# hccho2/Tacotron-Wavenet-Vocoder-Korean

Measured on AMD Instinct MI355X. Metric: WaveNet autoregressive audio samples/sec at 24 kHz, batch=8, higher is better.
Workload: dtype f32

## Files before the change

### tacotron-wavenet-vocoder-korean_amd/csrc/twv_wavenet_xcd.hip

```cpp
#include <hip/hip_runtime.h>
#include <stdint.h>
#include <string>
#include <type_traits>
#include "../../include/twv_amd.h"
#include "twv_layout.hpp"
#include "twv_math.hpp"
#include "twv_dev.hpp"
#include "twv_dpp.hpp"
#include "twv_categorical.hpp"
#include "twv_xcd.hpp"

using namespace twv;

#ifndef TWV_CHAIN_PAD
#define TWV_CHAIN_PAD 0
#endif
#ifndef TWV_WATCHDOG_LOG2
#define TWV_WATCHDOG_LOG2 21
#endif
#define TWV_STR2(x) #x
#define TWV_STR(x) TWV_STR2(x)
namespace {

typedef __attribute__((address_space(1))) unsigned long long gu64;
#define LDSU64(i) (((__attribute__((address_space(3))) volatile unsigned long long*)lds)[(i)])

typedef unsigned u32x2v __attribute__((ext_vector_type(2)));
typedef unsigned u32x4s __attribute__((ext_vector_type(4)));
constexpr int kAuxLoad = (int)(16u | 0x80000000u), kAuxStore = 0;
#ifndef TWV_XCD_KF
#define TWV_XCD_KF 1
#endif

__device__ __forceinline__ unsigned long long xb_load(rsrc_t rs, int uword, int lword)
{
    asm volatile("" ::: "memory");
    const u32x2v v = __builtin_amdgcn_raw_buffer_load_b64(rs, lword * 8, uword * 8, kAuxLoad);
    return ((unsigned long long)v.y << 32) | (unsigned long long)v.x;
}
__device__ __forceinline__ u32x4s xb_load2(rsrc_t rs, int uword, int lpair)
{
    asm volatile("" ::: "memory");
    return __builtin_amdgcn_raw_buffer_load_b128(rs, lpair * 16, uword * 8, kAuxLoad);
}
template <bool BAR> __device__ __forceinline__ unsigned long long xb_load_t(rsrc_t rs, int uword, int lword)
{
    if (BAR) asm volatile("" ::: "memory");
    return xb_load(rs, uword, lword);
}
__device__ __forceinline__ unsigned long long xbm_load(rsrc_t rs, int uword, int lword) { return xb_load_t<true>(rs, uword, lword); }
__device__ __forceinline__ u32x4s xbm_load2(rsrc_t rs, int uword, int lpair)
{
    asm volatile("" ::: "memory");
    return xb_load2(rs, uword, lpair);
}
__device__ __forceinline__ void xb_store(rsrc_t rs, int uword, int lword, unsigned tag, float v)
{
    __builtin_amdgcn_raw_buffer_store_b64(u32x2v{__float_as_uint(v), tag}, rs, lword * 8, uword * 8, kAuxStore);
    asm volatile("" ::: "memory");
}
__device__ __forceinline__ void xb_store2(rsrc_t rs, int uword, int lane, unsigned tag, float va, float vb)
{
    const u32x4s d = {__float_as_uint(va), tag, __float_as_uint(vb), tag};
    __builtin_amdgcn_raw_buffer_store_b128(d, rs, lane * 16, uword * 8, kAuxStore);
    asm volatile("s_nop 1" ::"v"(d) : "memory");
}
__device__ __forceinline__ unsigned g_tag(unsigned long long q) { return (unsigned)(q >> 32); }
__device__ __forceinline__ float g_val(unsigned long long q) { return __uint_as_float((unsigned)q); }

struct Poll {
    rsrc_t rs;
    int* status;
    int it;
    bool dead;
};
template <bool BAR = false>
__device__ __forceinline__ bool poll_tick(Poll& p, int code)
{
    if (p.dead) return false;
    if (((++p.it) & 63) == 0) {
        if (xb_load_t<BAR>(p.rs, (int)XcdExch::CTRL + 1, 0) != 0ull) { p.dead = true; return false; }
        if (p.it > (1 << TWV_WATCHDOG_LOG2)) {
            atomicMax(p.status, code);
            xb_store(p.rs, (int)XcdExch::CTRL + 1, 0, 1u, 0.0f);
            p.dead = true;
            return false;
        }
    }
    return true;
}
__device__ __forceinline__ void nap_until(unsigned long long target)
{
#pragma nounroll
    for (int i = 0; i < 4096 && __builtin_amdgcn_s_memtime() < target; ++i) __builtin_amdgcn_s_sleep(8);
}

__device__ __forceinline__ int lane_of_z(int k) { return ((k & 2) ? 16 : 0) + 2 * (k >> 2) + (k & 1); }
__device__ __forceinline__ int lane_of_x(int j) { return j < 16 ? j : 16 + j; }

struct ChainRegs { float wc[32]; float bd; };

#define XSTAMP(cond_, slot_) do { if ((INSTR & 1) && a.prof != nullptr && b == a.prof_stream && t < a.prof_steps && lane == 0 && (cond_)) a.prof[(long long)t * 64 + (slot_)] = wall_clock64(); } while (0)

#define WACC_DECL() unsigned long long wacc_[6] = {0, 0, 0, 0, 0, 0}, w0_ = 0, wt0_ = 0; if (INSTR & 4) wt0_ = __builtin_amdgcn_s_memtime()
#define WACC_T0() do { if (INSTR & 4) w0_ = __builtin_amdgcn_s_memtime(); } while (0)
#define WACC_T1(i_) do { if (INSTR & 4) wacc_[i_] += __builtin_amdgcn_s_memtime() - w0_; } while (0)
constexpr int kTraceStep = 2000;
#define WTRACE(cond_, slot_) do { if ((INSTR & 4) && a.prof != nullptr && t == kTraceStep && (cond_) && lane == 0) a.prof[2048 + (slot_)] = wall_clock64(); } while (0)
#define WACC_OUT(prof_, slot_, wave_) do { if ((INSTR & 4) && (prof_) != nullptr && (slot_) >= 0 && lane == 0) {                 \
        unsigned long long* o_ = (prof_) + (((slot_) * 8 + (wave_)) * 8);                                                        \
        o_[0] = __builtin_amdgcn_s_memtime() - wt0_;                                                                             \
        o_[1] = wacc_[0]; o_[2] = wacc_[1]; o_[3] = wacc_[2]; o_[4] = wacc_[3]; o_[5] = wacc_[4]; o_[6] = wacc_[5]; } } while (0)
#define XMARK(role_, stage_) do { if ((INSTR & 1) && lane == 0) xb_store(rs, (int)XcdExch::MARK + (role_) * 8 + (int)(threadIdx.x >> 6), 0, (unsigned)t + 1u, (float)(stage_)); } while (0)

enum { ROLE_CHAIN = 0, ROLE_SERVICE = 1, ROLE_SKIP0 = 2, ROLE_CONV0 = 10, ROLE_LC0 = 18 };
constexpr int kXcdStreamsPerXcd = kXcdStreams / 8;

struct XArgs {
    XcdLaunch p;
    int n_lc_wg, lc_lpw;
    int total_roles;
};

template <int NS> struct XStreams { rsrc_t rs[NS]; int b[NS]; };
__device__ __forceinline__ rsrc_t exch_rsrc(const XcdLaunch& a, int b)
{
    return __builtin_amdgcn_make_buffer_rsrc(a.exch + (long long)b * XcdExch::WORDS, 0, (int)(XcdExch::WORDS * 8), 0x00020000);
}
struct XLazyRs { const XcdLaunch* a; int xcc, ns; __device__ __forceinline__ rsrc_t operator[](int k) const { return exch_rsrc(*a, xcc + 8 * (k < ns ? k : 0)); } };
struct XLazyB { int xcc, ns; __device__ __forceinline__ int operator[](int k) const { return xcc + 8 * (k < ns ? k : 0); } };
template <int NS> struct XStreamsLazy { XLazyRs rs; XLazyB b; };
constexpr int kSkipLdsWords = 32 * 64;
constexpr int kConvLdsFloats = 16 * 64 + 64;

template <int INSTR, bool ALL, bool FORCED, bool SEG1, bool TWOSEG, int NC, bool ONEHOT = false, int HW = -1>
__device__ __forceinline__ void chain_role(const XArgs& xa, int b, rsrc_t rs)
{
    const XcdLaunch& a = xa.p;
    const Layout& L = a.lay;
    const int w = __builtin_amdgcn_readfirstlane(threadIdx.x >> 6), lane = threadIdx.x & 63;
    const int NL = L.NL, T = a.T;
    const bool use_bias = L.use_bias != 0, has_gc = L.G > 0, has_lc = L.L > 0;
    constexpr bool forced = FORCED;
    const int l0 = SEG1 ? kXcdSeg0Layers + 4 * w : (w < 6 ? 4 * w : 24 + 3 * (w - 6));
    const int lw0 = SEG1 ? 4 * w : l0;
    const int cap = SEG1 ? 4 : (w < 6 ? 4 : 3);
    int nl = NL - l0;
    nl = nl < 0 ? 0 : (nl > cap ? cap : nl);
    const int nlc = NC >= 0 ? NC : nl;
    const bool next_has = (l0 + nl < NL);
    const bool head = HW >= 0 ? (HW == 1) : (!SEG1 && (w == 7));
    const bool to_seg1 = TWOSEG && !SEG1 && w == 7 && next_has;
    constexpr bool two_seg = TWOSEG;
    if (nl == 0 && !head) return;
    const int oc = dpp_conv_out(lane), od = dpp_dense_out(lane);
    const ActCoef coef = act_coef(lane >= 32);
    float* stb = a.state + (long long)b * L.state_stride;
    Poll pl{rs, a.status, 0, false};
    constexpr int O_WD = 2048;

    ChainRegs W[4];
#pragma unroll
    for (int i = 0; i < 4; ++i) {
        if (i < nl) {
            const f32x4* src = reinterpret_cast<const f32x4*>(a.P + L.off_xl + (long long)(l0 + i) * kXcdXlFloats) + lane;
#pragma unroll
            for (int q = 0; q < 8; ++q) { const f32x4 v = src[q * 64]; W[i].wc[4 * q] = v.x; W[i].wc[4 * q + 1] = v.y; W[i].wc[4 * q + 2] = v.z; W[i].wc[4 * q + 3] = v.w; }
#pragma unroll
            for (int q = 0; q < 4; ++q) LDS4((O_WD >> 2) + ((lw0 + i) * 4 + q) * 64 + lane) = src[(8 + q) * 64];
            const f32x4 v = src[12 * 64];
            W[i].bd = dense_bias_init(lane, use_bias ? v.y : 0.0f);
        }
    }
    float ha = 0.0f, hb = 0.0f, first_in = 0.0f, b2v = 0.0f, s_lnl = 0.0f, s_tq = 0.0f, samp = 0.0f;
    float cp[4] = {0.0f, 0.0f, 0.0f, 0.0f};
    int q_prev = 0, q_valid = 0, samp_q = 0, first_q = 0;
    float w0row = 0.0f;
    double u_next = 0.0;
    const int chx = dpp_dense_out(lane);
    const bool sampler = head && !forced;
    const bool is15 = (lane & 15) == 15;
    auto causal_prepare = [&]() {
        const float t1 = __int_as_float(__builtin_amdgcn_update_dpp(0, __float_as_int(ha), 0x101, 0xf, 0xf, true));
        const float b0 = __int_as_float(__builtin_amdgcn_update_dpp(0, __float_as_int(hb), 0x150, 0xf, 0xf, true));
        ha = is15 ? b0 : t1;
        hb = __int_as_float(__builtin_amdgcn_update_dpp(0, __float_as_int(hb), 0x101, 0xf, 0xf, true));
        causal_partial_dpp(W[3].wc, ha, hb, cp);
    };
    auto noise = [&](int t) {
        const float* up = a.uniforms + ((long long)b * T + t) * (L.nr_mix + 1);
        const float u = lane <= L.nr_mix ? up[lane] : 0.5f;
        s_lnl = log_e(-log_e(u));
        const float uu = __shfl(u, L.nr_mix);
        s_tq = log_e(uu) - log_e(1.0f - uu);
    };
    if (head) {
        if constexpr (ONEHOT) {
            const int* meta = reinterpret_cast<const int*>(stb + L.st_meta);
            q_valid = __builtin_amdgcn_readfirstlane(meta[M_PREV_VALID]);
            q_prev = __builtin_amdgcn_readfirstlane(meta[M_QPREV]) & (L.Q - 1);
            w0row = a.P[L.off_causal + (long long)q_prev * 32 + chx];
            if (!forced) first_q = reinterpret_cast<const int*>(a.first_input)[b];
        } else {
            const f32x4* src = reinterpret_cast<const f32x4*>(a.P + L.off_xc) + lane;
#pragma unroll
            for (int q = 0; q < 8; ++q) { const f32x4 v = src[q * 64]; W[3].wc[4 * q] = v.x; W[3].wc[4 * q + 1] = v.y; W[3].wc[4 * q + 2] = v.z; W[3].wc[4 * q + 3] = v.w; }
            ha = stb[L.st_hist + (lane & 15)];
            hb = stb[L.st_hist + 16 + (lane & 15)];
            if (!forced) first_in = reinterpret_cast<const float*>(a.first_input)[b];
            if (sampler && use_bias && lane < L.O) b2v = a.P[L.off_b2 + lane];
            causal_prepare();
        }
// ... 41 lines not shown
            if (lane == 0) {
                if (sampler && t > 0) a.out[(long long)b * T + t - 1] = samp;
                xb_store(rs, (int)XcdExch::CTRL, 0, tag, 0.0f);
            }
            hb = is15 ? s_in : hb;
            if (t + 1 < T) causal_prepare();
            if (sampler) noise(t);
            }
            __builtin_amdgcn_s_setprio(0);
        }
        XMARK(SEG1 ? 30 : ROLE_CHAIN, 1);
        float pre[4] = {0.0f, 0.0f, 0.0f, 0.0f};
        if (nlc > 0) {
            pl.it = 0;
            for (;;) {
                bool ok = true;
#pragma unroll
                for (int i = 0; i < 4; ++i) {
                    if (i < nlc) {
                        const unsigned long long qp = xb_load(rs, (int)XcdExch::PG + (l0 + i) * 64, oc);
                        ok = ok && g_tag(qp) == tag;
                        pre[i] = g_val(qp);
                    }
                }
                if (__all(ok)) break;
                if (!poll_tick(pl, 31)) break;
                __builtin_amdgcn_s_sleep(4);
            }
            XSTAMP(!SEG1, 26 + w);
            XMARK(SEG1 ? 30 : ROLE_CHAIN, 2);
            if (in_period) nap_until(t_in + in_period - (in_period >> 4));
            unsigned long long q;
            pl.it = 0;
            if (SEG1 && w == 0) {
                for (;;) {
                    q = xb_load(rs, (int)XcdExch::SEG, lane);
                    if (__all(g_tag(q) == tag)) break;
                    if (!poll_tick(pl, 36)) break;
                }
            } else {
                for (;;) {
                    q = LDSU64(w * 64 + lane);
                    if (__all(g_tag(q) == tag)) break;
                    if (!poll_tick(pl, 33)) break;
                }
            }
            __builtin_amdgcn_s_setprio(3);
            X = g_val(q);
            now_in = __builtin_amdgcn_s_memtime();
            XSTAMP(true, (SEG1 ? 40 : 2) + w);
            XMARK(SEG1 ? 30 : ROLE_CHAIN, 3);
        }
        constexpr bool DEFER = ALL && !FORCED && !SEG1 && NC > 0 && HW == 0;
        float zs[4] = {0.0f, 0.0f, 0.0f, 0.0f}, xs[4] = {0.0f, 0.0f, 0.0f, 0.0f};
        auto run_layers = [&](auto nc) {
            constexpr int N = decltype(nc)::value;
#pragma unroll
            for (int i = 0; i < N; ++i) {
                float wd[16];
#pragma unroll
                for (int q = 0; q < 4; ++q) {
                    const f32x4 v = LDS4((O_WD >> 2) + ((lw0 + i) * 4 + q) * 64 + lane);
                    wd[4 * q] = v.x; wd[4 * q + 1] = v.y; wd[4 * q + 2] = v.z; wd[4 * q + 3] = v.w;
                }
                const float z = layer_front_dpp(W[i].wc, coef, X, pre[i]);
                if (DEFER) { zs[i] = z; xs[i] = X; }
                else xb_store2(rs, (int)XcdExch::ZX + (l0 + i) * 128, lane, tag, z, X);
                layer_back_dpp(wd, W[i].bd, z, X);
                if ((INSTR & 2) && a.dbg != nullptr && t < a.dbg_steps) {
                    float* dp = a.dbg + ((long long)b * a.dbg_steps + t) * ((long long)NL * 64 + L.Opad) + (long long)(l0 + i) * 64;
                    if (lane < 32) dp[dpp_z_index(lane)] = z;
                    if ((lane & 16) == 0) dp[32 + od] = X;
                }
            }
        };
        if constexpr (NC > 0) run_layers(std::integral_constant<int, NC>{});
        else {
            if (nl == 4) run_layers(std::integral_constant<int, 4>{});
            else if (nl == 3) run_layers(std::integral_constant<int, 3>{});
            else if (nl == 2) run_layers(std::integral_constant<int, 2>{});
            else if (nl == 1) run_layers(std::integral_constant<int, 1>{});
        }
        if (to_seg1) xb_store(rs, (int)XcdExch::SEG, lane, tag, X);
        else if (nlc > 0) LDSU64((next_has ? w + 1 : 9) * 64 + lane) = ((unsigned long long)tag << 32) | (unsigned long long)__float_as_uint(X);
        XSTAMP(DEFER && nl > 0, (SEG1 ? 48 : 10) + w);
        if (DEFER) {
#pragma unroll
            for (int i = 0; i < (NC > 0 ? NC : 0); ++i) xb_store2(rs, (int)XcdExch::ZX + (l0 + i) * 128, lane, tag, zs[i], xs[i]);
        }
        if (forced && nl > 0 && !next_has) {
            if (SEG1) xb_store(rs, (int)XcdExch::DONE, lane, tag, 0.0f);
            else LDSU64(8 * 64 + lane) = (unsigned long long)tag << 32;
        }
        if (nlc > 0) {
            const unsigned long long d = now_in - t_in;
            in_period = (t_in != 0 && d < (1ull << 18)) ? d : 0;
            t_in = now_in;
        }
        if (!sampler) __builtin_amdgcn_s_setprio(0);
        XSTAMP(!DEFER && nl > 0, (SEG1 ? 48 : 10) + w);
        XMARK(SEG1 ? 30 : ROLE_CHAIN, 4);
        if constexpr (ONEHOT) {
          if (sampler) {
            __builtin_amdgcn_s_setprio(3);
            u32x4s d0, d1;
            pl.it = 0;
            for (;;) {
                d0 = xb_load2(rs, (int)XcdExch::QL, lane * 2);
                d1 = xb_load2(rs, (int)XcdExch::QL, lane * 2 + 1);
                if (__all(d0.y == tag && d0.w == tag && d1.y == tag && d1.w == tag)) break;
                if (!poll_tick(pl, 34)) break;
            }
            XSTAMP(true, 18);
            XMARK(SEG1 ? 30 : ROLE_CHAIN, 5);
            const float y[4] = {__uint_as_float(d0.x), __uint_as_float(d0.z), __uint_as_float(d1.x), __uint_as_float(d1.z)};
            if ((INSTR & 2) && a.dbg != nullptr && t < a.dbg_steps) {
#pragma unroll
                for (int k = 0; k < 4; ++k)
                    a.dbg[((long long)b * a.dbg_steps + t) * ((long long)NL * 64 + L.Opad) + (long long)NL * 64 + lane + 64 * k] = y[k];
            }
            bool bad_p = false;
            samp_q = categorical_sample<4>(y, L.Q, lane, a.temperature, u_next, nullptr,
                                           ((INSTR & 1) && a.prof != nullptr && b == a.prof_stream && t < a.prof_steps) ? a.prof + (long long)t * 64 + 38 : nullptr, &bad_p);
            if (bad_p && lane == 0) atomicMax(a.status, 31);
            XSTAMP(true, 19);
          }
        } else
        if (sampler) {
            __builtin_amdgcn_s_setprio(3);
            const int half = lane >> 5;
            unsigned long long q[8];
            pl.it = 0;
            for (;;) {
                bool good = true;
#pragma unroll
                for (int k = 0; k < 4; ++k) {
                    const u32x4s d = xb_load2(rs, (int)XcdExch::PT, (half * 4 + k) * 32 + (lane & 31));
                    q[2 * k] = ((unsigned long long)d.y << 32) | d.x;
                    q[2 * k + 1] = ((unsigned long long)d.w << 32) | d.z;
                    good = good && d.y == tag && d.w == tag;
                }
                if (__all(good)) break;
                if (!poll_tick(pl, 34)) break;
            }
            XSTAMP(true, 18);
            XMARK(SEG1 ? 30 : ROLE_CHAIN, 5);
            float y = g_val(q[0]);
#pragma unroll
            for (int k = 1; k < 8; ++k) y = y + g_val(q[k]);
#pragma unroll
            for (int k = 0; k < 8; ++k) {
                const auto sw = __builtin_amdgcn_permlane32_swap((unsigned)q[k], (unsigned)q[k], false, false);
                y = y + __uint_as_float(sw[1]);
// ... 327 lines not shown
                        if (!summer) __builtin_amdgcn_s_sleep(1);
                    }
                    if ((INSTR & 1) && pl.dead && g == 0 && lane == 0) {
                        xb_store(rs, (int)XcdExch::MARK + 176 + v * 4, 0, g_tag(qz), __uint_as_float(g_tag(qz)));
                        xb_store(rs, (int)XcdExch::MARK + 177 + v * 4, 0, (unsigned)l, __uint_as_float((unsigned)pl.it));
                        xb_store(rs, (int)XcdExch::MARK + 178 + v * 4, 0, tag, __uint_as_float((unsigned)si));
                    }
                    if (!anysum && k == 0) {
                        const unsigned long long now = __builtin_amdgcn_s_memtime();
                        if (si == 0) { const unsigned long long d = now - seen[0]; period = (seen[0] != 0 && d < (1ull << 18)) ? d : 0; }
                        seen[si] = now;
                    }
                    XSTAMP(g == 0 && summer && l == NL - 1, 20);
                    const auto sw = __builtin_amdgcn_permlane32_swap((unsigned)qz, (unsigned)qz, false, false);
                    float val = dot(__uint_as_float(sw[0]), __uint_as_float(sw[1]));
                    if (use_bias) val = val + bias;
                    if (!summer) {
                        LDSU64(k * SW + l * 64 + lane) = ((unsigned long long)tag << 32) | (unsigned long long)__float_as_uint(val);
                    } else {
                        drain(true);
                        tot[k] = (l == 0) ? val : tot[k] + val;
                        nextl[k] = l + 1;
                        if (l == NL - 1 && !pl.dead) {
                            const float h = (KF > 0 || tot[k] > 0.0f) ? tot[k] : 0.0f;
                            xb_store(rs, (int)XcdExch::H1 + g * 64, lane, tag, h);
                            XSTAMP(g == 0, 21);
                        }
                    }
                }
            }
        };
#pragma unroll
        for (int j = 0; j < kLds; ++j) {
            if (j < nlds && !pl.dead)
                own_layer([&](float xa_, float xb_) __attribute__((always_inline)) { return dot32_dpp_lds(o_tile4 + (v + 8 * j) * (kTile / 4), lane, xa_, xb_); }, bs[j], v + 8 * j, j, 0, NS);
        }
#pragma unroll
        for (int i = 0; i < kReg; ++i) {
            if (i < nown && !pl.dead) {
                const int l = NLDS + v + 8 * i;
                own_layer([&](float xa_, float xb_) __attribute__((always_inline)) { return dot32_dpp(ws[i].w, xa_, xb_); }, bs[kLds + i], l, kLds + i, 0,
                          (SPLIT && vB >= 0 && l == NL - 1) ? 2 : NS);
            }
        }
        if (SPLIT && sumB && !pl.dead)
            own_layer([&](float xa_, float xb_) __attribute__((always_inline)) { return dot32_dpp(wx.w, xa_, xb_); }, bx, NL - 1, kSlots, 2, NS);
    }
    if (pl.dead && lane == 0) {
#pragma unroll
        for (int k = 0; k < NS; ++k) xb_store(sx.rs[k], (int)XcdExch::CTRL + 1, 0, 1u, 0.0f);
    }
}

template <int KF, bool BAR>
__device__ __forceinline__ unsigned long long conv1_fetch_h1(Poll& pl, const rsrc_t rs, const int v, const int lane, const unsigned tag, const int last_layer,
                                                             const int zc_lane, const float (&wl)[32], const float bl, const bool use_bias, bool& saw_z)
{
    unsigned long long q;
    pl.it = 0;
    if (KF > 0) {
        unsigned long long qz;
        float val = 0.0f;
        bool havez = false;
        for (;;) {
            if (!havez) qz = xb_load_t<BAR>(rs, (int)XcdExch::ZX + last_layer * 128, zc_lane * 2);
            q = xb_load_t<BAR>(rs, (int)XcdExch::H1 + v * 64, lane);
            if (!havez && __all(g_tag(qz) == tag)) {
                const auto sw = __builtin_amdgcn_permlane32_swap((unsigned)qz, (unsigned)qz, false, false);
                val = dot32_dpp(wl, __uint_as_float(sw[0]), __uint_as_float(sw[1]));
                if (use_bias) val = val + bl;
                havez = true;
                saw_z = true;
            }
            if (havez && __all(g_tag(q) == tag)) break;
            if (!poll_tick<BAR>(pl, 61)) break;
            if (!havez) __builtin_amdgcn_s_sleep(1);
        }
        const float tot = g_val(q) + val;
        const float h = tot > 0.0f ? tot : 0.0f;
        q = (unsigned long long)__float_as_uint(h);
    } else {
        for (;;) {
            q = xb_load_t<BAR>(rs, (int)XcdExch::H1 + v * 64, lane);
            if (__all(g_tag(q) == tag)) break;
            if (!poll_tick<BAR>(pl, 61)) break;
            __builtin_amdgcn_s_sleep(1);
        }
    }
    return q;
}
__device__ __forceinline__ void conv1_load_last_skip(const XcdLaunch& a, const int v, const int lane, Tile& wl, float& bl)
{
    const Layout& L = a.lay;
    const long long lb = L.off_layer0 + (long long)(L.NL - 1) * L.layer_stride;
    load_tile(wl, a.P + lb + LayerOff::SK + (long long)v * kTile, lane);
    if (L.use_bias != 0) bl = a.P[lb + LayerOff::SK + (long long)L.NSJ * kTile + v * 64 + lane];
}

template <int INSTR, int NS, bool BAR = false, class SX = XStreams<NS>, int KF = 0>
__device__ __forceinline__ void conv1_role(const XArgs& xa, const SX& sx, int g, const int ns_rt = NS, const int prof_slot = -1)
{
    const XcdLaunch& a = xa.p;
    const Layout& L = a.lay;
    const int v = __builtin_amdgcn_readfirstlane(threadIdx.x >> 6), lane = threadIdx.x & 63;
    const int T = a.T, NCH = L.NCH;
    const bool use_bias = L.use_bias != 0;
    Poll pl{sx.rs[0], a.status, 0, false};
    constexpr int O_PART = 0, O_CNT = 16 * 64;
    if (threadIdx.x < NS) LDSI(threadIdx.x * kConvLdsFloats + O_CNT) = 0;
    __syncthreads();
    const int c0 = 2 * v, c1 = 2 * v + 1;
    Tile ta, tb;
    load_tile(ta, a.P + L.off_w1 + ((long long)g * NCH + c0) * kTile, lane);
    load_tile(tb, a.P + L.off_w1 + ((long long)g * NCH + c1) * kTile, lane);
    const bool summer = v < 2;
    float b1v = 0.0f;
    Tile t2;
    if (summer) {
        if (use_bias) b1v = a.P[L.off_b1 + g * 64 + lane];
        load_tile(t2, a.P + L.off_w2 + (long long)(2 * g + v) * kTile, lane);
    }
    Tile wl;
    float bl = 0.0f;
    if (KF > 0) conv1_load_last_skip(a, v, lane, wl, bl);
    const int zc_lane = lane_of_z((lane < 32 ? 0 : 16) + (lane & 15));
    unsigned long long t_arr = 0, period = 0;
    WACC_DECL();
    for (int t = 0; t < T && !pl.dead; ++t) {
        asm volatile(".p2align 6");
        const unsigned tag = (unsigned)t + 1u;
        WACC_T0();
        if (period) nap_until(t_arr + period - (period >> 3));
        WACC_T1(0);
#pragma unroll
        for (int k = 0; k < NS; ++k) {
            if (pl.dead) break;
            if (k >= ns_rt) break;
            const rsrc_t rs = sx.rs[k];
            const int b = sx.b[k];
            const int ob = k * kConvLdsFloats;
            pl.rs = rs;
            XMARK(ROLE_CONV0 + g, 1);
            WACC_T0();
            bool saw_z = false;
            const unsigned long long q = conv1_fetch_h1<KF, BAR>(pl, rs, v, lane, tag, L.NL - 1, zc_lane, wl.w, bl, use_bias, saw_z);
            (void)saw_z;
            WACC_T1(1);
            WTRACE(prof_slot >= 0 && k == 0, 400 + g * 8 + v);
            unsigned long long now_arr = 0;
            if (k == 0) now_arr = __builtin_amdgcn_s_memtime();
            XSTAMP(g == 0 && v == 0, 22);
            const unsigned hq = (unsigned)q;
            const auto p16 = __builtin_amdgcn_permlane16_swap(hq, hq, false, false);
            const auto pa = __builtin_amdgcn_permlane32_swap(p16[0], p16[0], false, false);
            const auto pb = __builtin_amdgcn_permlane32_swap(p16[1], p16[1], false, false);
            float r0, r1;
            dot32_dpp_x2(ta.w, __uint_as_float(pa[0]), __uint_as_float(pb[0]), tb.w, __uint_as_float(pa[1]), __uint_as_float(pb[1]), r0, r1);
            lds[ob + O_PART + c0 * 64 + lane] = r0;
            lds[ob + O_PART + c1 * 64 + lane] = r1;
            asm volatile("" ::: "memory");
            if (lane == 0) __hip_atomic_fetch_add(&LDSI(ob + O_CNT), 1, __ATOMIC_RELAXED, __HIP_MEMORY_SCOPE_WORKGROUP);
            if (k == 0) {
                const unsigned long long d = now_arr - t_arr;
                period = (t_arr != 0 && d < (1ull << 18)) ? d : 0;
                t_arr = now_arr;
            }
            XSTAMP(g == 0 && v == 0, 23);
            XMARK(ROLE_CONV0 + g, 2);
            if (summer) {
                WACC_T0();
                pl.it = 0;
                while (LDSVI(ob + O_CNT) < 8 * (t + 1)) { if (!poll_tick<BAR>(pl, 62)) break; }
                WACC_T1(2);
                asm volatile("" ::: "memory");
                XSTAMP(g == 0 && v == 0, 24);
                float cp[16];
#pragma unroll
                for (int ch = 0; ch < 16; ++ch) cp[ch] = lds[ob + O_PART + ch * 64 + lane];
                __builtin_amdgcn_sched_barrier(0);
                float r = cp[0];
#pragma unroll
                for (int ch = 1; ch < 16; ++ch) r = r + cp[ch];
                if (use_bias) r = r + b1v;
                const float h = r > 0.0f ? r : 0.0f;
                const float p = (v == 0) ? dot_readlane_pipe(t2, h) : dot_readlane_pipe32(t2, h);
                if (lane < 32) xb_store(rs, (int)XcdExch::PT, (g * 32 + lane) * 2 + v, tag, p);
                WTRACE(prof_slot >= 0 && k == 0, 480 + g * 2 + v);
                XSTAMP(g == 0 && v == 0, 25);
            }
        }
    }
    if (pl.dead && lane == 0) {
#pragma unroll
        for (int k = 0; k < NS; ++k) xb_store(sx.rs[k], (int)XcdExch::CTRL + 1, 0, 1u, 0.0f);
    }
    WACC_OUT(a.prof, prof_slot, v);
}

constexpr int kConvQLdsFloats = 16 * 64 + 64 + 8 * 64;
template <int INSTR, int NS, int KF = 0>
__device__ __forceinline__ void conv1_onehot_role(const XArgs& xa, const XStreams<NS>& sx, int g)
{
    const XcdLaunch& a = xa.p;
    const Layout& L = a.lay;
    const int v = __builtin_amdgcn_readfirstlane(threadIdx.x >> 6), lane = threadIdx.x & 63;
    const int T = a.T, NCH = L.NCH;
    const bool use_bias = L.use_bias != 0;
    Poll pl{sx.rs[0], a.status, 0, false};
    constexpr int O_PART = 0, O_CNT = 16 * 64, O_P2 = 16 * 64 + 64;
    if (threadIdx.x < NS) { LDSI(threadIdx.x * kConvQLdsFloats + O_CNT) = 0; LDSI(threadIdx.x * kConvQLdsFloats + O_CNT + 1) = 0; }
    __syncthreads();
    const int c0 = 2 * v, c1 = 2 * v + 1;
    Tile ta, tb;
    load_tile(ta, a.P + L.off_w1 + ((long long)g * NCH + c0) * kTile, lane);
    load_tile(tb, a.P + L.off_w1 + ((long long)g * NCH + c1) * kTile, lane);
    float w2[32];
    {
        const int ch2 = lane < 32 ? c0 : c1;
        const f32x4* src = reinterpret_cast<const f32x4*>(a.P + L.off_w2 + ((long long)(g >> 1) * NCH + ch2) * kTile) + ((g & 1) * 32 + (lane & 31));
#pragma unroll
        for (int q = 0; q < 8; ++q) { const f32x4 w = src[q * 64]; w2[4 * q] = w.x; w2[4 * q + 1] = w.y; w2[4 * q + 2] = w.z; w2[4 * q + 3] = w.w; }
    }
    float b1v = 0.0f, b2v = 0.0f;
    if (use_bias && v == 0) b1v = a.P[L.off_b1 + g * 64 + lane];
    if (use_bias && v == 1 && lane < 32) b2v = a.P[L.off_b2 + g * 32 + lane];
    Tile wl;
    float bl = 0.0f;
    if (KF > 0) conv1_load_last_skip(a, v, lane, wl, bl);
    const int zc_lane = lane_of_z((lane < 32 ? 0 : 16) + (lane & 15));
    const int cls = g * 32 + (lane & 31);
    const int ql_word = (cls & 63) * 4 + (cls >> 6);
    unsigned long long t_arr = 0, period = 0;
    for (int t = 0; t < T && !pl.dead; ++t) {
        asm volatile(".p2align 6");
        const unsigned tag = (unsigned)t + 1u;
        if (period) nap_until(t_arr + period - (period >> 3));
#pragma unroll
        for (int k = 0; k < NS; ++k) {
            if (pl.dead) break;
            const rsrc_t rs = sx.rs[k];
            const int ob = k * kConvQLdsFloats;
            const int b = sx.b[k];
            (void)b;
            pl.rs = rs;
            bool saw_z = false;
            unsigned long long q = conv1_fetch_h1<KF, false>(pl, rs, v, lane, tag, L.NL - 1, zc_lane, wl.w, bl, use_bias, saw_z);
            (void)saw_z;
            unsigned long long now_arr = 0;
            if (k == 0) now_arr = __builtin_amdgcn_s_memtime();
            XSTAMP(g == 0 && v == 0, 22);
            {
                const unsigned hq = (unsigned)q;
                const auto p16 = __builtin_amdgcn_permlane16_swap(hq, hq, false, false);
                const auto pa = __builtin_amdgcn_permlane32_swap(p16[0], p16[0], false, false);
                const auto pb = __builtin_amdgcn_permlane32_swap(p16[1], p16[1], false, false);
                float r0, r1;
                dot32_dpp_x2(ta.w, __uint_as_float(pa[0]), __uint_as_float(pb[0]), tb.w, __uint_as_float(pa[1]), __uint_as_float(pb[1]), r0, r1);
                lds[ob + O_PART + c0 * 64 + lane] = r0;
                lds[ob + O_PART + c1 * 64 + lane] = r1;
            }
            asm volatile("" ::: "memory");
            if (lane == 0) __hip_atomic_fetch_add(&LDSI(ob + O_CNT), 1, __ATOMIC_RELAXED, __HIP_MEMORY_SCOPE_WORKGROUP);
            if (k == 0) {
                const unsigned long long d = now_arr - t_arr;
                period = (t_arr != 0 && d < (1ull << 18)) ? d : 0;
                t_arr = now_arr;
            }
            XSTAMP(g == 0 && v == 0, 23);
            if (v == 0) {
                pl.it = 0;
                while (LDSVI(ob + O_CNT) < 8 * (t + 1)) { if (!poll_tick(pl, 62)) break; }
                asm volatile("" ::: "memory");
                XSTAMP(g == 0, 24);
                float cp[16];
#pragma unroll
                for (int ch = 0; ch < 16; ++ch) cp[ch] = lds[ob + O_PART + ch * 64 + lane];
                __builtin_amdgcn_sched_barrier(0);
                float r = cp[0];
#pragma unroll
                for (int ch = 1; ch < 16; ++ch) r = r + cp[ch];
                if (use_bias) r = r + b1v;
                const float h = r > 0.0f ? r : 0.0f;
                xb_store(rs, (int)XcdExch::H2 + g * 64, lane, tag, h);
                XSTAMP(g == 0, 25);
            }
            pl.it = 0;
            for (;;) {
                q = xb_load(rs, (int)XcdExch::H2 + v * 64, lane);
                if (__all(g_tag(q) == tag)) break;
                if (!poll_tick(pl, 63)) break;
                __builtin_amdgcn_s_sleep(1);
            }
            XSTAMP(g == 0 && v == 1, 34);
            {
                const unsigned hq = (unsigned)q;
                const auto p16 = __builtin_amdgcn_permlane16_swap(hq, hq, false, false);
                const float r2 = dot32_dpp(w2, __uint_as_float(p16[0]), __uint_as_float(p16[1]));
                lds[ob + O_P2 + v * 64 + lane] = r2;
            }
            asm volatile("" ::: "memory");
// ... 190 lines not shown
        if (hdr[XH_MAGIC] != kXcdCondMagic || (unsigned)hdr[XH_MODE] > (unsigned)XLC_MEL) {
            atomicMax(a.status, 74);
            atomicCAS(decision, 0, 2);
        }
        if (atomicAdd(arrived, 1) + 1 == xa.total_roles) atomicCAS(decision, 0, 1);
        int f = 0;
#pragma nounroll
        for (int i = 0; i < (1 << 15); ++i) {
            f = atomicAdd(decision, 0);
            if (f != 0) break;
            __builtin_amdgcn_s_sleep(32);
        }
        if (f == 0) {
            const int old = atomicCAS(decision, 0, 2);
            f = old == 0 ? 2 : old;
            if (old == 0) atomicMax(a.status, 90);
        }
        s_go = (f == 1) ? 1 : 0;
    }
    __syncthreads();
    return s_go != 0;
}

template <int INSTR, bool BIGK, bool ONE, bool ONEHOT = false>
__global__ void __launch_bounds__(512) wn_xcd_generate_kernel(XArgs xa)
{
    const XcdLaunch& a = xa.p;
    unsigned xcc;
    asm volatile("s_getreg_b32 %0, hwreg(HW_REG_XCC_ID)" : "=s"(xcc));
    xcc &= 15u;
    int ticket = 0;
    if (threadIdx.x == 0) ticket = (xcc < (unsigned)a.B && xcc < 8u) ? atomicAdd(a.roles + xcc, 1) : 1 << 20;
    ticket = __shfl(ticket, 0);
    __shared__ int s_ticket;
    if (threadIdx.x == 0) s_ticket = ticket;
    for (int i = threadIdx.x; i < kXcdStreamsPerXcd * kSkipLdsWords * 2 + 64; i += blockDim.x) lds[i] = 0.0f;
    __syncthreads();
    ticket = s_ticket;
    const int ns = xcc < (unsigned)a.B && xcc < 8u ? (a.B - (int)xcc + 7) / 8 : 0;
    constexpr int nseg = BIGK ? 2 : 1;
    const int nchain = ns * nseg;
    if (ticket >= nchain + ns + 16 + xa.n_lc_wg) return;
    if (!roles_resident(xa)) return;
    const bool forced = a.forced != nullptr;
    auto exch_of = [&](int b) { return __builtin_amdgcn_make_buffer_rsrc(a.exch + (long long)b * XcdExch::WORDS, 0, (int)(XcdExch::WORDS * 8), 0x00020000); };
    if (ticket < nchain + ns) {
        const int k = ticket < nchain ? ticket / nseg : ticket - nchain;
        const int b = (int)xcc + 8 * k;
        const rsrc_t rs = exch_of(b);
        if (ticket < nchain) {
            if (ticket % nseg == 0) {
                const int wv = __builtin_amdgcn_readfirstlane(threadIdx.x >> 6);
                const int nlw = a.lay.NL - (wv < 6 ? 4 * wv : 24 + 3 * (wv - 6));
                if (forced) chain_role<INSTR, true, true, false, BIGK, -1, ONEHOT>(xa, b, rs);
                else if (nlw >= 4 && wv < 6) chain_role<INSTR, true, false, false, BIGK, 4, ONEHOT, 0>(xa, b, rs);
                else if (nlw >= 3 && wv == 6) chain_role<INSTR, true, false, false, BIGK, 3, ONEHOT, 0>(xa, b, rs);
                else if (nlw >= 3 && wv == 7) chain_role<INSTR, true, false, false, BIGK, 3, ONEHOT, 1>(xa, b, rs);
                else chain_role<INSTR, true, false, false, BIGK, -1, ONEHOT>(xa, b, rs);
            } else if constexpr (BIGK) {
                const int wv = __builtin_amdgcn_readfirstlane(threadIdx.x >> 6);
                if (forced) chain_role<INSTR, true, true, true, true, -1>(xa, b, rs);
                else if (a.lay.NL - kXcdSeg0Layers - 4 * wv >= 4) chain_role<INSTR, true, false, true, true, 4>(xa, b, rs);
                else chain_role<INSTR, true, false, true, true, -1>(xa, b, rs);
            }
        }
        else service_role<INSTR, BIGK>(xa, b, rs);
        return;
    }
    const int role = ticket - nchain - ns;
    auto shared_roles = [&](auto nsc) {
        constexpr int NS = decltype(nsc)::value;
        XStreams<NS> sx;
#pragma unroll
        for (int k = 0; k < NS; ++k) { sx.b[k] = (int)xcc + 8 * k; sx.rs[k] = exch_of(sx.b[k]); }
        constexpr int KF = TWV_XCD_KF;
        constexpr bool kUnfolded = KF == 0 || INSTR == 0;
        const bool fold = KF > 0 && (a.lay.NL > KF || !kUnfolded);
        if (role < 8) {
            if (!forced) {
                if (fold) skip_role<INSTR, NS, BIGK, KF>(xa, sx, role);
                else if constexpr (kUnfolded) skip_role<INSTR, NS, BIGK, 0>(xa, sx, role);
            }
        }
        else if (role < 16) {
            if (!forced) {
                if constexpr (ONEHOT) {
                    if (fold) conv1_onehot_role<INSTR, NS, KF>(xa, sx, role - 8);
                    else if constexpr (kUnfolded) conv1_onehot_role<INSTR, NS, 0>(xa, sx, role - 8);
                }
                else if (fold) conv1_role<INSTR, NS, false, XStreams<NS>, KF>(xa, sx, role - 8);
                else if constexpr (kUnfolded) conv1_role<INSTR, NS>(xa, sx, role - 8);
            }
        }
        else lc_role<INSTR, NS, BIGK>(xa, sx, role - 16);
    };
    if constexpr (BIGK) {
        if (ns == 1) shared_roles(std::integral_constant<int, 1>{});
        else shared_roles(std::integral_constant<int, 2>{});
    } else if constexpr (ONE) {
        shared_roles(std::integral_constant<int, 1>{});
    } else {
        if (ns == 1) shared_roles(std::integral_constant<int, 1>{});
        else if (ns == 2) shared_roles(std::integral_constant<int, 2>{});
        else if (ns == 3) shared_roles(std::integral_constant<int, 3>{});
        else shared_roles(std::integral_constant<int, 4>{});
    }
}

#define MMARK(rs_, slot_, stage_) do { if ((INSTR & 2) && lane == 0) xb_store(rs_, (int)XcdExch::MARK + (slot_), 0, (unsigned)t + 1u, (float)(stage_)); } while (0)
constexpr int kMS = 2;
constexpr int kManyChains = 6;
constexpr int kManyPerXcd = kMS * kManyChains;
constexpr int kM_BOX = 10;
constexpr int kM_OWD = 4096;
constexpr int kM_OGC = kM_OWD + kXcdSeg0Layers * 1024;
constexpr int kM_OHS = kM_OGC + kMS * kXcdSeg0Layers * 64;
// ... 852 lines not shown
namespace twv {

bool xcd_model_ok(const Layout& L)
{
    const bool head_ok = L.scalar ? (L.ifw == 32 && L.O <= 32 && L.NOJ == 1) : (L.Q == 256 && L.O == 256);
    return head_ok && L.S == 512 && L.NL >= 1 && L.NL <= kXcdMaxLayers && L.NLC <= 4;
}
static bool xcd_many_lc_fits(const Layout& L) { return (long long)kManyPerXcd * (L.n_up + 1) * L.NLC * 32 <= kManyLds / 8; }
int xcd_max_streams(const Layout& L) { return L.NL > kXcdSeg0Layers ? kXcdStreams / 2 : (L.scalar && xcd_many_lc_fits(L) ? kXcdManyStreams : kXcdStreams); }
static int lc_layers_per_wave(const Layout& L) { const int n = L.NLC > 0 ? (L.NL > kXcdSeg0Layers ? 6 : 4) / L.NLC : 1; return n < 1 ? 1 : (n > 4 ? 4 : n); }
int xcd_lc_workgroups(const Layout& L)
{
    if (L.L == 0) return 0;
    const int lpw = lc_layers_per_wave(L);
    const int waves = (L.NL + lpw - 1) / lpw;
    return (waves + 7) / 8;
}
int xcd_workgroups_per_stream(const Layout& L) { return ROLE_LC0 + xcd_lc_workgroups(L); }
size_t xcd_exchange_bytes(int batch) { return (size_t)batch * XcdExch::WORDS * 8 + 64; }
void xcd_pack(float* packed, const float* blob, const Layout& L, hipStream_t st)
{
    hipLaunchKernelGGL(wn_xcd_pack_kernel, dim3(512), dim3(256), 0, st, packed, blob, L);
}
bool xcd_uses_many(const Layout& L, int batch, int many_opt)
{
    return L.scalar && (batch > kXcdStreams || many_opt == 1 || (many_opt == 0 && batch >= kXcdManyFrom)) && L.NL <= kXcdSeg0Layers && xcd_many_lc_fits(L);
}
int xcd_launch(const XcdLaunch& p, hipStream_t st)
{
    XArgs xa;
    xa.p = p;
    xa.n_lc_wg = xcd_lc_workgroups(p.lay);
    xa.lc_lpw = lc_layers_per_wave(p.lay);
    const bool many = xcd_uses_many(p.lay, p.B, p.many);
    xa.total_roles = 0;
    for (int x = 0; x < 8 && x < p.B; ++x) {
        const int ns = (p.B - x + 7) / 8;
        if (many) xa.total_roles += 2 * ((ns + kMS - 1) / kMS) + 16 + xa.n_lc_wg;
        else xa.total_roles += ns * (p.lay.NL > kXcdSeg0Layers ? 2 : 1) + ns + 16 + xa.n_lc_wg;
    }
    const size_t shm = many ? (size_t)kManyLds * 4 : p.lay.NL > kXcdSeg0Layers ? (size_t)159 * 1024 : (size_t)(2048 + 32 * 1024) * 4;
    int dev = 0, cus = 256;
    hipDeviceProp_t prop;
    if (hipGetDevice(&dev) == hipSuccess && hipGetDeviceProperties(&prop, dev) == hipSuccess) cus = prop.multiProcessorCount;
    else (void)hipGetLastError();
    const int grid = 2 * cus;
    const int instr = (p.prof != nullptr ? 1 : 0) | (p.dbg != nullptr ? 2 : 0);
    auto go = [&](auto kern) {
        (void)hipFuncSetAttribute((const void*)kern, hipFuncAttributeMaxDynamicSharedMemorySize, (int)shm);
        (void)hipGetLastError();
        hipLaunchKernelGGL(kern, dim3(grid), dim3(512), shm, st, xa);
    };
    if (!many && instr != 0 && p.lay.NL <= TWV_XCD_KF)
        return twv_fail(TWV_E_UNSUPPORTED, "layer dumps / phase stamps of the XCD kernel need a model of at least two layers (set option \"xcd\" = 0 for the generic kernel)");
    if (many) {
        if (p.B > kXcdManyStreams) return twv_fail(TWV_E_UNSUPPORTED, "the many-streams XCD kernel takes at most 96 streams");
        if (instr == 3) return twv_fail(TWV_E_UNSUPPORTED, "layer dumps and wait accounting are separate builds of the many-streams kernel");
        if (instr == 1) go(wn_xcd_many_kernel<4>);
        else if (instr == 2) go(wn_xcd_many_kernel<2>);
        else go(wn_xcd_many_kernel<0>);
    }
    else if (!p.lay.scalar) {
        if (p.B > (p.lay.NL > kXcdSeg0Layers ? kXcdStreams / 2 : kXcdStreams)) return twv_fail(TWV_E_UNSUPPORTED, "the one-hot XCD kernel takes at most 32 streams (16 above 30 layers)");
        if (instr == 3 || (instr != 0 && p.lay.NL > kXcdSeg0Layers))
            return twv_fail(TWV_E_UNSUPPORTED, "the one-hot XCD kernel has layer dumps OR phase stamps, up to 30 layers (set option \"xcd\" = 0 for the generic kernel)");
        if (p.lay.NL > kXcdSeg0Layers) go(wn_xcd_generate_kernel<0, true, false, true>);
        else if (instr == 2) go(wn_xcd_generate_kernel<2, false, false, true>);
        else if (instr == 1) go(wn_xcd_generate_kernel<1, false, false, true>);
        else if (p.B <= 8) go(wn_xcd_generate_kernel<0, false, true, true>);
        else go(wn_xcd_generate_kernel<0, false, false, true>);
    }
    else if (p.lay.NL > kXcdSeg0Layers) {
        if (instr != 0) return twv_fail(TWV_E_UNSUPPORTED, "layer dumps / phase stamps exist for the 30-layer XCD kernel only (set option \"xcd\" = 0 for the generic kernel)");
        go(wn_xcd_generate_kernel<0, true, false>);
    }
    else if (instr == 3) go(wn_xcd_generate_kernel<3, false, false>);
    else if (instr == 2) go(wn_xcd_generate_kernel<2, false, false>);
    else if (instr == 1) go(wn_xcd_generate_kernel<1, false, false>);
    else if (p.B <= 8) go(wn_xcd_generate_kernel<0, false, true>);
    else go(wn_xcd_generate_kernel<0, false, false>);
    const hipError_t e = hipGetLastError();
    if (e != hipSuccess) return twv_fail(TWV_E_HIP, std::string("xcd launch: ") + hipGetErrorString(e));
    return TWV_OK;
}

}
```

### tacotron-wavenet-vocoder-korean_amd/csrc/twv_xcd.hpp

```cpp
#pragma once
#include <hip/hip_runtime.h>
#include <stddef.h>
#include <stdint.h>
#include "twv_layout.hpp"

namespace twv {

constexpr int kXcdSeg0Layers = 30;
constexpr int kXcdMaxLayers = 50;
constexpr int kXcdLs = 64;
constexpr int kXcdStreams = 32;
constexpr int kXcdManyFrom = 21;
constexpr int kXcdManyStreams = 96;
constexpr int kXcdLcRing = 16;
#ifndef TWV_MANY_LC_RING
#define TWV_MANY_LC_RING 8
#endif
constexpr int kXcdManyLcRing = TWV_MANY_LC_RING;
constexpr int kXcdXlFloats = 13 * 64 * 4;
constexpr int kXcdXcFloats = 8 * 64 * 4;

enum { XH_MAGIC = 0, XH_MODE = 1, XH_ROWS = 2, XH_WORDS = 64 };
constexpr int kXcdCondMagic = 0x58434431;
enum { XLC_NONE = 0, XLC_UPSAMPLED = 1, XLC_MEL = 2 };

struct XcdExch {
    static constexpr long long ZX = 0;
    static constexpr long long PG = ZX + kXcdLs * 128;
    static constexpr long long LG = PG + kXcdLs * 64;
    static constexpr long long H1 = LG + kXcdLs * 64;
    static constexpr long long PT = H1 + 512;
    static constexpr long long LCR = PT + 512;
    static constexpr long long CTRL = LCR + (long long)kXcdLcRing * kXcdLs * 64;
    static constexpr long long MARK = CTRL + 64;
    static constexpr long long SEG = MARK + 256;
    static constexpr long long DONE = SEG + 64;
    static constexpr long long SKT = DONE + 64;
    static constexpr long long H2 = SKT + 3 * 2 * 256;
    static constexpr long long QL = H2 + 512;
    static constexpr long long WORDS = QL + 256;
};

struct XcdLaunch {
    const float* P;
    float* state;
    const float* cond;
    const void* first_input;
    const void* forced;
    const float* uniforms;
    float temperature;
    float* out;
    int* status;
    float* dbg;
    int dbg_steps;
    unsigned long long* prof;
    int prof_steps;
    int prof_stream;
    int B, T;
    int many;
    unsigned long long* exch;
    int* roles;
    Layout lay;
};

bool xcd_model_ok(const Layout& L);
int xcd_max_streams(const Layout& L);
bool xcd_uses_many(const Layout& L, int batch, int many_opt);
int xcd_lc_workgroups(const Layout& L);
int xcd_workgroups_per_stream(const Layout& L);
size_t xcd_exchange_bytes(int batch);
int xcd_launch(const XcdLaunch& a, hipStream_t st);
void xcd_pack(float* packed, const float* blob, const Layout& L, hipStream_t st);

}
```

Measured before the change: 938,000.

## Generalize skip-fold in conv1 to the last KF layers via packed z area

Replaces the single-last-layer skip fold in the conv1 roles with a generalized fold over the last KF layers. Chain waves store those layers' z values into a new packed exchange area (ZF), and conv1 computes their skip contributions directly. The chain dispatch gains FOLD variants that publish fold-layer z early and defer the normal ZX stores. The aim is to take the tail layers' skip accumulation off the critical path. With the default KF=1 the behaviour is similar to before but uses the new layout and adds extra stores.

```diff
diff --git a/tacotron-wavenet-vocoder-korean_amd/csrc/twv_wavenet_xcd.hip b/tacotron-wavenet-vocoder-korean_amd/csrc/twv_wavenet_xcd.hip
--- a/tacotron-wavenet-vocoder-korean_amd/csrc/twv_wavenet_xcd.hip
+++ b/tacotron-wavenet-vocoder-korean_amd/csrc/twv_wavenet_xcd.hip
@@ -31,6 +31,7 @@
 #ifndef TWV_XCD_KF
 #define TWV_XCD_KF 1
 #endif
+static_assert(TWV_XCD_KF >= 0 && TWV_XCD_KF <= 4, "the packed z area XcdExch::ZF holds four layers");
 
 __device__ __forceinline__ unsigned long long xb_load(rsrc_t rs, int uword, int lword)
 {
@@ -97,6 +98,13 @@
 
 __device__ __forceinline__ int lane_of_z(int k) { return ((k & 2) ? 16 : 0) + 2 * (k >> 2) + (k & 1); }
 __device__ __forceinline__ int lane_of_x(int j) { return j < 16 ? j : 16 + j; }
+__device__ __forceinline__ int zf_word(int j) { return 32 * (j >> 1) + (j & 1); }
+__device__ __forceinline__ int zf_chain_lane(int lane)
+{
+    if (lane >= 32) return 128 + 2 * (lane - 32);
+    const int c = lane & 15, k = 4 * (c >> 1) + 2 * (lane >> 4) + (c & 1);
+    return 64 * (k >> 4) + 2 * (k & 15);
+}
 
 struct ChainRegs { float wc[32]; float bd; };
 
@@ -133,7 +141,7 @@
 constexpr int kSkipLdsWords = 32 * 64;
 constexpr int kConvLdsFloats = 16 * 64 + 64;
 
-template <int INSTR, bool ALL, bool FORCED, bool SEG1, bool TWOSEG, int NC, bool ONEHOT = false, int HW = -1>
+template <int INSTR, bool ALL, bool FORCED, bool SEG1, bool TWOSEG, int NC, bool ONEHOT = false, int HW = -1, int FOLD = 0>
 __device__ __forceinline__ void chain_role(const XArgs& xa, int b, rsrc_t rs)
 {
     const XcdLaunch& a = xa.p;
@@ -158,6 +166,10 @@
     float* stb = a.state + (long long)b * L.state_stride;
     Poll pl{rs, a.status, 0, false};
     constexpr int O_WD = 2048;
+    constexpr int KF = TWV_XCD_KF;
+    static_assert(FOLD != 1 || NC > 0, "FOLD 1 needs the layer count at compile time");
+    const int fb = (KF > 0 && NL > KF) ? NL - KF : NL;
+    const int zf_lane = zf_chain_lane(lane);
 
     ChainRegs W[4];
 #pragma unroll
@@ -305,6 +317,8 @@
             XMARK(SEG1 ? 30 : ROLE_CHAIN, 3);
         }
         constexpr bool DEFER = ALL && !FORCED && !SEG1 && NC > 0 && HW == 0;
+        constexpr bool LATE = DEFER || FOLD != 0;
+        bool fz[4] = {false, false, false, false};
         float zs[4] = {0.0f, 0.0f, 0.0f, 0.0f}, xs[4] = {0.0f, 0.0f, 0.0f, 0.0f};
         auto run_layers = [&](auto nc) {
             constexpr int N = decltype(nc)::value;
@@ -317,7 +331,10 @@
                     wd[4 * q] = v.x; wd[4 * q + 1] = v.y; wd[4 * q + 2] = v.z; wd[4 * q + 3] = v.w;
                 }
                 const float z = layer_front_dpp(W[i].wc, coef, X, pre[i]);
-                if (DEFER) { zs[i] = z; xs[i] = X; }
+                if constexpr (FOLD == 1) fz[i] = i >= NC - KF;
+                else if constexpr (FOLD == 2) fz[i] = l0 + i >= fb;
+                if (fz[i]) xb_store(rs, (int)XcdExch::ZF + zf_word(FOLD == 1 ? i - (NC - KF) : l0 + i - fb), zf_lane, tag, z);
+                if (DEFER || fz[i]) { zs[i] = z; xs[i] = X; }
                 else xb_store2(rs, (int)XcdExch::ZX + (l0 + i) * 128, lane, tag, z, X);
                 layer_back_dpp(wd, W[i].bd, z, X);
                 if ((INSTR & 2) && a.dbg != nullptr && t < a.dbg_steps) {
@@ -336,10 +353,15 @@
         }
         if (to_seg1) xb_store(rs, (int)XcdExch::SEG, lane, tag, X);
         else if (nlc > 0) LDSU64((next_has ? w + 1 : 9) * 64 + lane) = ((unsigned long long)tag << 32) | (unsigned long long)__float_as_uint(X);
-        XSTAMP(DEFER && nl > 0, (SEG1 ? 48 : 10) + w);
+        XSTAMP(LATE && nl > 0, (SEG1 ? 48 : 10) + w);
         if (DEFER) {
 #pragma unroll
             for (int i = 0; i < (NC > 0 ? NC : 0); ++i) xb_store2(rs, (int)XcdExch::ZX + (l0 + i) * 128, lane, tag, zs[i], xs[i]);
+        }
+        if constexpr (FOLD != 0) {
+#pragma unroll
+            for (int i = 0; i < 4; ++i)
+                if (fz[i]) xb_store2(rs, (int)XcdExch::ZX + (l0 + i) * 128, lane, tag, zs[i], xs[i]);
         }
         if (forced && nl > 0 && !next_has) {
             if (SEG1) xb_store(rs, (int)XcdExch::DONE, lane, tag, 0.0f);
@@ -351,7 +373,7 @@
             t_in = now_in;
         }
         if (!sampler) __builtin_amdgcn_s_setprio(0);
-        XSTAMP(!DEFER && nl > 0, (SEG1 ? 48 : 10) + w);
+        XSTAMP(!LATE && nl > 0, (SEG1 ? 48 : 10) + w);
         XMARK(SEG1 ? 30 : ROLE_CHAIN, 4);
         if constexpr (ONEHOT) {
           if (sampler) {
@@ -785,31 +807,43 @@
     }
 }
 
-template <int KF, bool BAR>
-__device__ __forceinline__ unsigned long long conv1_fetch_h1(Poll& pl, const rsrc_t rs, const int v, const int lane, const unsigned tag, const int last_layer,
-                                                             const int zc_lane, const float (&wl)[32], const float bl, const bool use_bias, bool& saw_z)
+template <int KF> struct FoldTiles { Tile w[KF > 0 ? KF : 1]; float b[KF > 0 ? KF : 1]; };
+template <int KF, bool BAR, bool ST = false>
+__device__ __forceinline__ unsigned long long conv1_fetch_h1(Poll& pl, const rsrc_t rs, const int v, const int lane, const unsigned tag,
+                                                             const FoldTiles<KF>& ft, const bool use_bias, unsigned long long* st)
 {
     unsigned long long q;
     pl.it = 0;
-    if (KF > 0) {
-        unsigned long long qz;
-        float val = 0.0f;
-        bool havez = false;
+    if constexpr (KF > 0) {
+        const int r = (lane >> 4) & 1;
+        float s[KF];
+        unsigned have = 0;
+        u32x4s d = {0u, 0u, 0u, 0u};
         for (;;) {
-            if (!havez) qz = xb_load_t<BAR>(rs, (int)XcdExch::ZX + last_layer * 128, zc_lane * 2);
+            if (have != (1u << KF) - 1u) d = xb_load2(rs, (int)XcdExch::ZF, lane);
             q = xb_load_t<BAR>(rs, (int)XcdExch::H1 + v * 64, lane);
-            if (!havez && __all(g_tag(qz) == tag)) {
-                const auto sw = __builtin_amdgcn_permlane32_swap((unsigned)qz, (unsigned)qz, false, false);
-                val = dot32_dpp(wl, __uint_as_float(sw[0]), __uint_as_float(sw[1]));
-                if (use_bias) val = val + bl;
-                havez = true;
-                saw_z = true;
-            }
-            if (havez && __all(g_tag(q) == tag)) break;
+#pragma unroll
+            for (int j = 0; j < KF; ++j) {
+                if (have & (1u << j)) continue;
+                if (!__all(r != (j >> 1) || ((j & 1) ? d.w : d.y) == tag)) break;
+                const unsigned zz = (j & 1) ? d.z : d.x;
+                const auto p16 = __builtin_amdgcn_permlane16_swap(zz, zz, false, false);
+                const unsigned zr = (j >> 1) ? p16[1] : p16[0];
+                const auto sw = __builtin_amdgcn_permlane32_swap(zr, zr, false, false);
+                float val = dot32_dpp(ft.w[j].w, __uint_as_float(sw[0]), __uint_as_float(sw[1]));
+                if (use_bias) val = val + ft.b[j];
+                s[j] = val;
+                have |= 1u << j;
+                if (ST && j == KF - 1) st[0] = wall_clock64();
+            }
+            if (have == (1u << KF) - 1u && __all(g_tag(q) == tag)) break;
             if (!poll_tick<BAR>(pl, 61)) break;
-            if (!havez) __builtin_amdgcn_s_sleep(1);
-        }
-        const float tot = g_val(q) + val;
+            if (have != (1u << KF) - 1u) __builtin_amdgcn_s_sleep(1);
+        }
+        if (ST) st[1] = wall_clock64();
+        float tot = g_val(q);
+#pragma unroll
+        for (int j = 0; j < KF; ++j) tot = tot + s[j];
         const float h = tot > 0.0f ? tot : 0.0f;
         q = (unsigned long long)__float_as_uint(h);
     } else {
@@ -822,13 +856,19 @@
     }
     return q;
 }
-__device__ __forceinline__ void conv1_load_last_skip(const XcdLaunch& a, const int v, const int lane, Tile& wl, float& bl)
+template <int KF>
+__device__ __forceinline__ void conv1_load_fold_skip(const XcdLaunch& a, const int v, const int lane, FoldTiles<KF>& ft)
 {
     const Layout& L = a.lay;
-    const long long lb = L.off_layer0 + (long long)(L.NL - 1) * L.layer_stride;
-    load_tile(wl, a.P + lb + LayerOff::SK + (long long)v * kTile, lane);
-    if (L.use_bias != 0) bl = a.P[lb + LayerOff::SK + (long long)L.NSJ * kTile + v * 64 + lane];
-}
+#pragma unroll
+    for (int j = 0; j < KF; ++j) {
+        const long long lb = L.off_layer0 + (long long)(L.NL - KF + j) * L.layer_stride;
+        load_tile(ft.w[j], a.P + lb + LayerOff::SK + (long long)v * kTile, lane);
+        ft.b[j] = L.use_bias != 0 ? a.P[lb + LayerOff::SK + (long long)L.NSJ * kTile + v * 64 + lane] : 0.0f;
+    }
+}
+#define XSTAMP_FOLD(cond_) do { if ((INSTR & 1) && a.prof != nullptr && b == a.prof_stream && t < a.prof_steps && lane == 0 && (cond_)) { \
+        a.prof[(long long)t * 64 + 56] = fst[0]; a.prof[(long long)t * 64 + 57] = fst[1]; } } while (0)
 
 template <int INSTR, int NS, bool BAR = false, class SX = XStreams<NS>, int KF = 0>
 __device__ __forceinline__ void conv1_role(const XArgs& xa, const SX& sx, int g, const int ns_rt = NS, const int prof_slot = -1)
@@ -853,10 +893,8 @@
         if (use_bias) b1v = a.P[L.off_b1 + g * 64 + lane];
         load_tile(t2, a.P + L.off_w2 + (long long)(2 * g + v) * kTile, lane);
     }
-    Tile wl;
-    float bl = 0.0f;
-    if (KF > 0) conv1_load_last_skip(a, v, lane, wl, bl);
-    const int zc_lane = lane_of_z((lane < 32 ? 0 : 16) + (lane & 15));
+    FoldTiles<KF> ft;
+    if constexpr (KF > 0) conv1_load_fold_skip<KF>(a, v, lane, ft);
     unsigned long long t_arr = 0, period = 0;
     WACC_DECL();
     for (int t = 0; t < T && !pl.dead; ++t) {
@@ -875,9 +913,9 @@
             pl.rs = rs;
             XMARK(ROLE_CONV0 + g, 1);
             WACC_T0();
-            bool saw_z = false;
-            const unsigned long long q = conv1_fetch_h1<KF, BAR>(pl, rs, v, lane, tag, L.NL - 1, zc_lane, wl.w, bl, use_bias, saw_z);
-            (void)saw_z;
+            unsigned long long fst[2] = {0, 0};
+            const unsigned long long q = conv1_fetch_h1<KF, BAR, (INSTR & 1) != 0 && KF != 0>(pl, rs, v, lane, tag, ft, use_bias, fst);
+            XSTAMP_FOLD(g == 0 && v == 0 && KF != 0);
             WACC_T1(1);
             WTRACE(prof_slot >= 0 && k == 0, 400 + g * 8 + v);
             unsigned long long now_arr = 0;
@@ -957,10 +995,8 @@
     float b1v = 0.0f, b2v = 0.0f;
     if (use_bias && v == 0) b1v = a.P[L.off_b1 + g * 64 + lane];
     if (use_bias && v == 1 && lane < 32) b2v = a.P[L.off_b2 + g * 32 + lane];
-    Tile wl;
-    float bl = 0.0f;
-    if (KF > 0) conv1_load_last_skip(a, v, lane, wl, bl);
-    const int zc_lane = lane_of_z((lane < 32 ? 0 : 16) + (lane & 15));
+    FoldTiles<KF> ft;
+    if constexpr (KF > 0) conv1_load_fold_skip<KF>(a, v, lane, ft);
     const int cls = g * 32 + (lane & 31);
     const int ql_word = (cls & 63) * 4 + (cls >> 6);
     unsigned long long t_arr = 0, period = 0;
@@ -976,9 +1012,9 @@
             const int b = sx.b[k];
             (void)b;
             pl.rs = rs;
-            bool saw_z = false;
-            unsigned long long q = conv1_fetch_h1<KF, false>(pl, rs, v, lane, tag, L.NL - 1, zc_lane, wl.w, bl, use_bias, saw_z);
-            (void)saw_z;
+            unsigned long long fst[2] = {0, 0};
+            unsigned long long q = conv1_fetch_h1<KF, false, (INSTR & 1) != 0 && KF != 0>(pl, rs, v, lane, tag, ft, use_bias, fst);
+            XSTAMP_FOLD(g == 0 && v == 0 && KF != 0);
             unsigned long long now_arr = 0;
             if (k == 0) now_arr = __builtin_amdgcn_s_memtime();
             XSTAMP(g == 0 && v == 0, 22);
@@ -1275,16 +1311,20 @@
             if (ticket % nseg == 0) {
                 const int wv = __builtin_amdgcn_readfirstlane(threadIdx.x >> 6);
                 const int nlw = a.lay.NL - (wv < 6 ? 4 * wv : 24 + 3 * (wv - 6));
+                const int fb = a.lay.NL > TWV_XCD_KF ? a.lay.NL - TWV_XCD_KF : a.lay.NL;
                 if (forced) chain_role<INSTR, true, true, false, BIGK, -1, ONEHOT>(xa, b, rs);
-                else if (nlw >= 4 && wv < 6) chain_role<INSTR, true, false, false, BIGK, 4, ONEHOT, 0>(xa, b, rs);
-                else if (nlw >= 3 && wv == 6) chain_role<INSTR, true, false, false, BIGK, 3, ONEHOT, 0>(xa, b, rs);
-                else if (nlw >= 3 && wv == 7) chain_role<INSTR, true, false, false, BIGK, 3, ONEHOT, 1>(xa, b, rs);
-                else chain_role<INSTR, true, false, false, BIGK, -1, ONEHOT>(xa, b, rs);
+                else if (nlw >= 4 && wv < 6 && 4 * wv + 4 <= fb) chain_role<INSTR, true, false, false, BIGK, 4, ONEHOT, 0>(xa, b, rs);
+                else if (nlw >= 3 && wv == 6 && 27 <= fb) chain_role<INSTR, true, false, false, BIGK, 3, ONEHOT, 0>(xa, b, rs);
+                else if (nlw >= 3 && wv == 7 && !BIGK) chain_role<INSTR, true, false, false, BIGK, 3, ONEHOT, 1, 1>(xa, b, rs);
+                else if (nlw >= 3 && wv == 7 && fb >= kXcdSeg0Layers) chain_role<INSTR, true, false, false, BIGK, 3, ONEHOT, 1, 0>(xa, b, rs);
+                else chain_role<INSTR, true, false, false, BIGK, -1, ONEHOT, -1, 2>(xa, b, rs);
             } else if constexpr (BIGK) {
                 const int wv = __builtin_amdgcn_readfirstlane(threadIdx.x >> 6);
+                const int l0 = kXcdSeg0Layers + 4 * wv, fb = a.lay.NL > TWV_XCD_KF ? a.lay.NL - TWV_XCD_KF : a.lay.NL;
                 if (forced) chain_role<INSTR, true, true, true, true, -1>(xa, b, rs);
-                else if (a.lay.NL - kXcdSeg0Layers - 4 * wv >= 4) chain_role<INSTR, true, false, true, true, 4>(xa, b, rs);
-                else chain_role<INSTR, true, false, true, true, -1>(xa, b, rs);
+                else if (a.lay.NL - l0 >= 4 && l0 + 4 <= fb) chain_role<INSTR, true, false, true, true, 4, false, -1, 0>(xa, b, rs);
+                else if (a.lay.NL - l0 == 4) chain_role<INSTR, true, false, true, true, 4, false, -1, 1>(xa, b, rs);
+                else chain_role<INSTR, true, false, true, true, -1, false, -1, 2>(xa, b, rs);
             }
         }
         else service_role<INSTR, BIGK>(xa, b, rs);
@@ -2243,7 +2283,7 @@
         hipLaunchKernelGGL(kern, dim3(grid), dim3(512), shm, st, xa);
     };
     if (!many && instr != 0 && p.lay.NL <= TWV_XCD_KF)
-        return twv_fail(TWV_E_UNSUPPORTED, "layer dumps / phase stamps of the XCD kernel need a model of at least two layers (set option \"xcd\" = 0 for the generic kernel)");
+        return twv_fail(TWV_E_UNSUPPORTED, "layer dumps / phase stamps of the XCD kernel need a model of more than " TWV_STR(TWV_XCD_KF) " layers (set option \"xcd\" = 0 for the generic kernel)");
     if (many) {
         if (p.B > kXcdManyStreams) return twv_fail(TWV_E_UNSUPPORTED, "the many-streams XCD kernel takes at most 96 streams");
         if (instr == 3) return twv_fail(TWV_E_UNSUPPORTED, "layer dumps and wait accounting are separate builds of the many-streams kernel");
diff --git a/tacotron-wavenet-vocoder-korean_amd/csrc/twv_xcd.hpp b/tacotron-wavenet-vocoder-korean_amd/csrc/twv_xcd.hpp
--- a/tacotron-wavenet-vocoder-korean_amd/csrc/twv_xcd.hpp
+++ b/tacotron-wavenet-vocoder-korean_amd/csrc/twv_xcd.hpp
@@ -38,7 +38,8 @@
     static constexpr long long SKT = DONE + 64;
     static constexpr long long H2 = SKT + 3 * 2 * 256;
     static constexpr long long QL = H2 + 512;
-    static constexpr long long WORDS = QL + 256;
+    static constexpr long long ZF = QL + 256;
+    static constexpr long long WORDS = ZF + 256;
 };
 
 struct XcdLaunch {
```

Result: no change. 941,300 (median of 6 runs) (+0.4%).
